# tangxyw/RecAlgorithm

Measured on AMD Instinct MI355X. Metric: CTR examples/sec (train step fwd+bwd+TF1-Adam), batch 4096/GPU, 26 fields x emb16, higher is better.
Workload: dtype f32; 1 GPU; DCN 3-layer CrossNet + MLP 512,256,128; 26 fields x emb16; batch 4096/GPU; data_batches=32, global_batch=4096, fields=26, emb_dim=16, embedding_rows=2790871, launch=hipGraph replay, parallelism=single

## Files before the change

### recalgorithm_amd/_lib.py

```python
from __future__ import annotations

import ctypes
import os
import re

from . import _abi
from ._abi import RecalgoError

_HERE = os.path.dirname(os.path.abspath(__file__))
LIB_PATH = os.environ.get("RECALGO_HIP_LIB") or os.path.join(_HERE, "librecalgo_hip.so")

P = ctypes.c_void_p


def _versioned(header: str):
    abi = _abi.read(header)
    defines = [c for c in abi.constants if re.fullmatch(r"RECALGO_(?:[A-Z0-9]+_)?ABI_VERSION", c)]
    queries = [f for f in abi.functions if re.fullmatch(r"recalgo_(?:[a-z0-9]+_)?abi_version", f)]
    if len(defines) != 1 or queries != [defines[0].lower()]:
        raise RecalgoError(f"include/{header}: a header of HEADERS has exactly one RECALGO_[<KEY>_]ABI_VERSION define and the "
                           f"one function recalgo_[<key>_]abi_version of the same key; found {defines} and {queries}")
    abi.version, abi.version_query = abi.constants[defines[0]], queries[0]
    abi.label = defines[0][len("RECALGO_"):-len("_VERSION")].replace("_", " ")
    return abi


HEADERS = {h: _versioned(h) for h in ("recalgo.h", "recalgo_cgc.h", "recalgo_wide.h", "recalgo_bst.h",
                                              "recalgo_res.h")}
MORE_HEADERS = {"recalgo_dien.h": _versioned("recalgo_dien.h")}
SERVING_HEADERS = {h: _versioned(h) for h in ("recalgo_serve.h", "recalgo_metrics.h", "recalgo_sumstep.h",
                                                      "recalgo_ragged.h", "recalgo_afm.h", "recalgo_feed.h")}
ABI = HEADERS["recalgo.h"]
SIGNATURES = ABI.functions
STRUCTS = ABI.structs
CONSTANTS = ABI.constants
ABI_VERSION = ABI.version
_lib = None


def all_headers() -> dict:
    return {**HEADERS, **MORE_HEADERS}


def every_header() -> dict:
    return {**all_headers(), **SERVING_HEADERS}

# ... 38 lines not shown
```

### recalgorithm_amd/algorithm/DCN/dcn.py

```python
from __future__ import annotations

import os
from typing import Tuple

import torch

from ... import feature_column as fc
from ... import flags, nn, ops
from ...estimator import (Estimator, EvalSpec, ModeKeys, RunConfig, TrainSpec, train_and_evaluate)
from ...model_tail import finish_model_fn
from ...variables import variable_scope
from .. import _common as common
from ..utils import eval_input_fn, parse_example, train_input_fn
from .cross_layer import cross_network

flags.DEFINE_string("model_dir", "./model_dir", "Directory where model parameters, graph, etc are saved")
flags.DEFINE_string("output_dir", "./output_dir", "Directory where pb file are saved")
flags.DEFINE_string("train_data", "../../dataset/wechat_algo_data1/tfrecord/train.tfrecord", "Path to the train data")
flags.DEFINE_string("eval_data", "../../dataset/wechat_algo_data1/tfrecord/test.tfrecord", "Path to the evaluation data")
flags.DEFINE_string("vocabulary_dir", "../../dataset/wechat_algo_data1/vocabulary/", "Folder where the vocabulary file is stored")
flags.DEFINE_integer("num_epochs", 1, "Epoch of training phase")
flags.DEFINE_integer("train_steps", 10000, "Number of (global) training steps to perform")
flags.DEFINE_integer("shuffle_buffer_size", 10000, "Dataset shuffle buffer size")
flags.DEFINE_integer("num_parallel_readers", -1, "Number of parallel readers for training data")
# ... 51 lines not shown

def dcn_model_fn(features, labels, mode, params):
    with variable_scope("dense_input"):
        dense_cols = params.get("dense_feature_columns") or []
        dense_input = fc.input_layer(features, dense_cols) if dense_cols else None
    with variable_scope("category_input"):
        if dense_input is None and int(params["num_cross_layer"]) > 0:
            with ops.gather_feeds_cross() as lz:
                category_input = fc.input_layer(features, params["category_feature_columns"])
                lz.keep(category_input)
        else:
            category_input = fc.input_layer(features, params["category_feature_columns"])
    concat_all = category_input if dense_input is None else torch.cat([dense_input, category_input], dim=-1)

    join = nn.GradJoin() if int(params["num_cross_layer"]) > 0 and len(params["hidden_units"]) > 0 else None
    with variable_scope("cross_part"):
        cross_vec = cross_network(concat_all, params["num_cross_layer"], grad_join=join)
    ops.flush_lazy_gathers()

    with variable_scope("dnn_part"):
        dnn_vec = concat_all
        for i, unit in enumerate(params["hidden_units"]):
            dnn_vec = nn.dense(dnn_vec, unit, activation="relu", name=f"dnn_dense_{i}", grad_join=join if i == 0 else None,
                               last_hidden=(i == len(params["hidden_units"]) - 1))

    with variable_scope("output_part"):
        output = nn.concat([cross_vec, dnn_vec], axis=-1)
        logit = nn.dense(output, 1, activation=None)

    return finish_model_fn(mode, logit, labels, params,
                           predictions=lambda prob: {"logit": logit, "probabilities": prob})


def main(unused_argv):
    global total_feature_columns, label_feature_columns
    dense_cols, category_cols, label_feature_columns = create_feature_columns()
    total_feature_columns = dense_cols + category_cols
    params = {
        "category_feature_columns": category_cols,
# ... 46 lines not shown
```

### recalgorithm_amd/csrc/cross.hip

```cpp
#include "common.h"
#include "cross_bwd.h"

namespace {

constexpr int kFwdThreads = 256;
constexpr int kBwdThreads = 512;
constexpr int kBwdWaves = kBwdThreads / 64;
constexpr int kMaxPartialRows = 256;

using recalgo_cross::wave_sum_n;

struct GatherSrc {
    const int64_t* ids;
    const float4* arena;
    const int64_t* row_base;
    unsigned F, K4;
};

template <int NV, int L>
__global__ __launch_bounds__(kFwdThreads) void cross_stack_fwd_kernel(
    float* __restrict__ x0, unsigned x_stride, const float4* __restrict__ w,
    const float4* __restrict__ b, unsigned B, unsigned d4, float* __restrict__ out,
    unsigned out_stride, GatherSrc gs) {
    const unsigned lane = threadIdx.x & 63;
    const unsigned wave = (blockIdx.x * kFwdThreads + threadIdx.x) >> 6;
    const unsigned nwaves = (gridDim.x * kFwdThreads) >> 6;

    float4 wv[L][NV], Bv[NV];
    float red[2 * L];
#pragma unroll
    for (int v = 0; v < NV; ++v) Bv[v] = f4_zero();
#pragma unroll
    for (int l = 0; l < L; ++l) {
        float acc = 0.f;
#pragma unroll
        for (int v = 0; v < NV; ++v) {
            unsigned idx = lane + v * 64;
            wv[l][v] = idx < d4 ? w[l * d4 + idx] : f4_zero();
            acc += f4_dot(Bv[v], wv[l][v]);
            if (idx < d4) Bv[v] = f4_add(Bv[v], b[l * d4 + idx]);
        }
        red[L + l] = acc;
    }

    for (unsigned ex = wave; ex < B; ex += nwaves) {
        float4* xr = reinterpret_cast<float4*>(x0 + (size_t)ex * x_stride);
        float4 xv[NV];
        if (gs.ids != nullptr) {
            long long id[NV];
#pragma unroll
            for (int v = 0; v < NV; ++v) {
                const unsigned idx = lane + v * 64;
                id[v] = idx < d4 ? gs.ids[(size_t)ex * gs.F + idx / gs.K4] : -1;
            }
#pragma unroll
            for (int v = 0; v < NV; ++v) {
                const unsigned idx = lane + v * 64, f = idx / gs.K4, q = idx - f * gs.K4;
                xv[v] = id[v] >= 0 ? gs.arena[(size_t)(gs.row_base[f] + id[v]) * gs.K4 + q] : f4_zero();
                if (idx < d4) xr[idx] = xv[v];
            }
        } else {
#pragma unroll
            for (int v = 0; v < NV; ++v) {
                unsigned idx = lane + v * 64;
                xv[v] = idx < d4 ? xr[idx] : f4_zero();
            }
        }
        float r[2 * L];
#pragma unroll
        for (int l = 0; l < L; ++l) {
            float acc = 0.f;
#pragma unroll
            for (int v = 0; v < NV; ++v) acc += f4_dot(xv[v], wv[l][v]);
            r[l] = acc;
            r[L + l] = red[L + l];
        }
        wave_sum_n<2 * L>(r);
        float c = 1.f;
#pragma unroll
        for (int l = 0; l < L; ++l) c += fmaf(c, r[l], r[L + l]);
        float4* orow = reinterpret_cast<float4*>(out + (size_t)ex * out_stride);
#pragma unroll
        for (int v = 0; v < NV; ++v) {
            unsigned idx = lane + v * 64;
            if (idx < d4) orow[idx] = f4_fma(xv[v], c, Bv[v]);
        }
    }
}

template <int NV, int L>
__global__ __launch_bounds__(kBwdThreads) void cross_stack_bwd_kernel(
    const float* __restrict__ x0, unsigned x_stride, const float4* __restrict__ w,
    const float4* __restrict__ b, const float* __restrict__ g, unsigned g_stride,
    const float* __restrict__ g_x0_extra, unsigned B, unsigned d4, float* __restrict__ dx0,
    float* __restrict__ partials) {
    extern __shared__ __attribute__((aligned(16))) float smem[];
    recalgo_cross::cross_stack_bwd_block<NV, L, kBwdWaves>(x0, x_stride, w, b, g, g_stride, g_x0_extra, B, d4, dx0, partials, blockIdx.x,
                                                          gridDim.x, smem);
}

template <int NV>
__global__ __launch_bounds__(kFwdThreads) void cross_layer_fwd_kernel(
// ... 269 lines not shown
```

### recalgorithm_amd/csrc/dense.hip

```cpp
#include <cstdlib>

#include "common.h"
#include "cross_bwd.h"
#include "act.h"
#include "tile_v2.h"
#include "dropout.h"
#include "slab_sum.h"

namespace {

using f32x16 = __attribute__((ext_vector_type(16))) float;

constexpr int kThreads = 256;
constexpr int BM = 64, BN = 64, BK = 32;
constexpr int kLdRC = BK + 1;
constexpr int kLdRM = 64;
constexpr int kBufFloats = 64 * tv2::kLdRC;

struct Operand {
    const float* p;
    const float* mask;
    int ld;
    int vec;
    int bytes;
// ... 222 lines not shown
    Segment seg[2];
    int nseg;
    const float* bias;
    int relu;
    float* y;
    int ldy;
    int M, N;
    float* bn_partials;
    const float* act_alpha;
    int act_kind;
    float* z;
    int vec_store;
    recalgo_drop::Spec drop;
};

template <bool FAST>
__global__ __launch_bounds__(kThreads) void dense_fwd_kernel(FwdArgs P) {
    __shared__ __attribute__((aligned(16))) float As[kStages * kBufFloats];
    __shared__ __attribute__((aligned(16))) float Bs[kStages * kBufFloats];
    const int tn_count = (P.N + BN - 1) / BN;
    const int tile = xcd_swizzle(blockIdx.x, gridDim.x);
    const int m0 = (tile / tn_count) * BM, n0 = (tile % tn_count) * BN;
    f32x16 acc, acc1;
#pragma unroll
    for (int r = 0; r < 16; ++r) acc[r] = acc1[r] = 0.f;
    float4 unused = f4_zero();
    const int lane = threadIdx.x & 63, wave = threadIdx.x >> 6;
    const int hi = lane >> 5, l32 = lane & 31;
    const bool rowwise = FAST && P.vec_store && P.bn_partials == nullptr;
    const int c4 = n0 + (wave & 1) * 32 + (lane & 7) * 4;
    float4 bias4 = f4_zero();
    if (rowwise && P.bias && c4 < P.N) bias4 = *reinterpret_cast<const float4*>(P.bias + c4);
    for (int s = 0; s < P.nseg; ++s)
        tile_mainloop<true, false, FAST, false, false, false>(P.seg[s], m0, n0, P.M, P.N, 0, P.seg[s].n_red, As, Bs, acc, acc1, unused);
    acc += acc1;
    const int col = n0 + (wave & 1) * 32 + l32;
    const bool dropping = recalgo_drop::enabled(P.drop);
    const recalgo_drop::Key dkey = dropping ? recalgo_drop::make_key(P.drop) : recalgo_drop::Key{0u, 0u};
    if (rowwise) {
        const int r0 = m0 + (wave >> 1) * 32;
        tv2::tile_rows(As + wave * tv2::kTileScratch, acc, [&](int, int row, int, float4 v) {
            v = f4_add(v, bias4);
            if (P.relu) v = make_float4(fmaxf(v.x, 0.f), fmaxf(v.y, 0.f), fmaxf(v.z, 0.f), fmaxf(v.w, 0.f));
            if (r0 + row < P.M && c4 < P.N) {
                if (dropping) {
                    const float4 f = recalgo_drop::factor4(P.drop, dkey, (uint32_t)(r0 + row) * (uint32_t)P.N + (uint32_t)c4);
                    v = make_float4(v.x * f.x, v.y * f.y, v.z * f.z, v.w * f.w);
                }
                *reinterpret_cast<float4*>(P.y + (size_t)(r0 + row) * P.ldy + c4) = v;
            }
        });
        return;
    }
    if (P.bn_partials == nullptr) {
        if (col >= P.N) return;
        const float bv = P.bias ? P.bias[col] : 0.f;
#pragma unroll
        for (int r = 0; r < 16; ++r) {
            const int row = m0 + (wave >> 1) * 32 + (r & 3) + 8 * (r >> 2) + 4 * hi;
            if (row < P.M) {
                float v = acc[r] + bv;
                if (P.relu) v = fmaxf(v, 0.f);
                if (dropping) v *= recalgo_drop::factor(P.drop, dkey, (uint32_t)row * (uint32_t)P.N + (uint32_t)col);
                P.y[(size_t)row * P.ldy + col] = v;
            }
        }
// ... 41 lines not shown
#pragma unroll
    for (int r = 0; r < 16; ++r) {
        const int row = m0 + (wave >> 1) * 32 + (r & 3) + 8 * (r >> 2) + 4 * hi;
        const float dlt = vals[r] - mean;
        if (cok && row < P.M) q = fmaf(dlt, dlt, q);
    }
    q += __shfl_xor(q, 32, 64);
    __syncthreads();
    if (hi == 0) red[(wave >> 1) * 64 + cl] = q;
    __syncthreads();
    if ((wave >> 1) == 0 && hi == 0 && cok) {
        float* prow = P.bn_partials + (size_t)(m0 / BM) * 2 * P.N;
        prow[col] = mean;
        prow[P.N + col] = red[cl] + red[64 + cl];
    }
}

struct DgradArgs {
    Segment seg;
    const float* c_in;
    float beta;
    int ldc;
    float* dx;
    int lddx;
    int M, K;
    int accumulate;
    int tiles_per_block;
    int vec_store;
    const float* dx_mask;
    int ld_mask;
// ... 343 lines not shown
    P.seg[0] = Segment{operand(x, nullptr, ldx, M, K), operand(w, nullptr, N, K, N), K};
    P.seg[1] = Segment{operand(x2, nullptr, ldx2, M, K2), operand(w2, nullptr, N, K2, N), K2};
    P.nseg = x2 ? 2 : 1;
    P.bias = bias; P.relu = relu; P.y = y; P.ldy = ldy; P.M = M; P.N = N;
    P.bn_partials = bn_partials;
    P.act_alpha = act_alpha; P.act_kind = act_kind == RECALGO_ACT_NONE ? 0 : 1 + act_kind; P.z = z;
    P.vec_store = (aligned16(y) && ldy % 4 == 0 && N % 4 == 0 && (bias == nullptr || aligned16(bias))) ? 1 : 0;
    P.drop = recalgo_drop::from_abi(drop);
    const int grid = cdiv(M, BM) * cdiv(N, BN);
    const bool fast = fast_rc(P.seg[0].a, K) && fast_rm(P.seg[0].b, N) && fast_rc(P.seg[1].a, K2) && fast_rm(P.seg[1].b, N);
    if (fast) hipLaunchKernelGGL(dense_fwd_kernel<true>, dim3(grid), dim3(kThreads), 0, as_stream(stream), P);
    else hipLaunchKernelGGL(dense_fwd_kernel<false>, dim3(grid), dim3(kThreads), 0, as_stream(stream), P);
    RECALGO_RETURN_LAST();
}

static bool build_dgrad(DgradArgs& P, const float* g, int ldg, const float* y_mask, const float* w, int M, int N, int K,
                        const float* c_in, int ldc, float beta, float* dx, int lddx, int accumulate) {
    if (!(M >= 0 && N > 0 && K > 0 && dx != nullptr && lddx >= K)) return false;
    if (!(g != nullptr && ldg >= N && w != nullptr)) return false;
    if (!(c_in == nullptr || ldc >= K)) return false;
    P.seg = Segment{operand(g, y_mask, ldg, M, N), operand(w, nullptr, N, K, N), N};
    P.c_in = c_in; P.beta = beta; P.ldc = ldc; P.dx = dx; P.lddx = lddx; P.M = M; P.K = K; P.accumulate = accumulate;
    P.tiles_per_block = 1;
    P.bn_x = P.bn_mean = P.bn_rstd = nullptr; P.bn_partials = nullptr;
    P.vec_store = (aligned16(dx) && lddx % 4 == 0 && K % 4 == 0 && (c_in == nullptr || (aligned16(c_in) && ldc % 4 == 0))) ? 1 : 0;
    P.dx_mask = nullptr; P.ld_mask = 0;
    return true;
}
static bool dgrad_fast(const DgradArgs& P) { return fast_rc(P.seg.a, P.seg.n_red) && fast_rc(P.seg.b, P.seg.n_red); }

// ... 300 lines not shown
```

### recalgorithm_amd/csrc/tile_v2.h

```cpp
#pragma once
#include "common.h"

namespace tv2 {

using f32x16 = __attribute__((ext_vector_type(16))) float;

constexpr int kThreads = 256;
constexpr int BK = 32;
constexpr int kLdRC = 36;
constexpr int kStages = 3;
constexpr int kOOB = (int)0x80000000u;

struct Operand {
    const float* p;
    const float* mask;
    int ld;
    int bytes;
};

template <bool RC, int W>
struct Geom {
    static constexpr int T = 64 * W;
    static constexpr int kFloats = RC ? T * kLdRC : BK * T;
    static constexpr int kLoads = 2 * W;
// ... 44 lines not shown
            const int o = red[j] + c * BK < red_end ? off[j] + c * step_b : kOOB;
            st.v[j] = __builtin_bit_cast(float4, __builtin_amdgcn_raw_buffer_load_b128(rs, o, 0, 0));
            if constexpr (MASK) st.m[j] = __builtin_bit_cast(float4, __builtin_amdgcn_raw_buffer_load_b128(rm, o, 0, 0));
        }
    }
    static __device__ __forceinline__ float4 value(const StageRegs<MASK, G::kLoads>& st, int j) {
        if constexpr (MASK) return relu_mask4(st.v[j], st.m[j]);
        else return st.v[j];
    }
    static __device__ __forceinline__ void store(float* __restrict__ S, const StageRegs<MASK, G::kLoads>& st, int j) {
        const int u = threadIdx.x + kThreads * j;
        float* d;
        if constexpr (RC) d = S + (u >> 3) * kLdRC + (u & 7) * 4;
        else d = S + (u / G::U) * G::T + (u % G::U) * 4;
        *reinterpret_cast<float4*>(d) = value(st, j);
    }
};

template <int W>
struct Frag {
    float x[4][W];
};

template <bool RC, int W>
__device__ __forceinline__ void read_item(const float* __restrict__ S, int wb, int l32, int hi, int g, int item, Frag<W>& f) {
    if constexpr (RC) {
        const float4 q = *reinterpret_cast<const float4*>(S + (wb + 32 * item + l32) * kLdRC + 8 * g + 4 * hi);
        f.x[0][item] = q.x; f.x[1][item] = q.y; f.x[2][item] = q.z; f.x[3][item] = q.w;
    } else {
        const float* p = S + (8 * g + 4 * hi + item) * Geom<false, W>::T + wb + W * l32;
        if constexpr (W == 1) f.x[item][0] = p[0];
        else if constexpr (W == 2) { const float2 q = *reinterpret_cast<const float2*>(p); f.x[item][0] = q.x; f.x[item][1] = q.y; }
        else { const float4 q = *reinterpret_cast<const float4*>(p); f.x[item][0] = q.x; f.x[item][1] = q.y; f.x[item][2] = q.z; f.x[item][3] = q.w; }
    }
}
template <bool RC, int W> constexpr int frag_items() { return RC ? W : 4; }

template <bool RC, int W>
__device__ __forceinline__ int idx_of(int sub, int lane_idx) { return RC ? 32 * sub + lane_idx : W * lane_idx + sub; }

template <bool A_RC, bool B_RC, int WM, int WN, bool MASK_A, bool MASK_B, bool COLSUM, bool EXACT, bool TWO = false>
__device__ __forceinline__ void mainloop(const Operand& A, const Operand& B, int m0, int n0, int M, int N, int red_begin,
                                         int red_end, float* __restrict__ As, float* __restrict__ Bs,
                                         f32x16 (&acc)[WM][WN], float4& colsum, f32x16 (*accb)[WN] = nullptr) {
    using GA = Geom<A_RC, WM>;
    using GB = Geom<B_RC, WN>;
    using SA = Stager<A_RC, WM, MASK_A, EXACT>;
    using SB = Stager<B_RC, WN, MASK_B, EXACT>;
    constexpr int nLA = GA::kLoads, nLB = GB::kLoads, nL = nLA + nLB;
    constexpr int nFA = frag_items<A_RC, WM>(), nFB = frag_items<B_RC, WN>(), nF = nFA + nFB;
    constexpr int G = 4 * WM * WN;
    static_assert(nL <= G, "one load / store item per slot");
    const int lane = threadIdx.x & 63, wave = threadIdx.x >> 6;
    const int hi = lane >> 5, l32 = lane & 31;
    const int wbA = (wave >> 1) * 32 * WM, wbB = (wave & 1) * 32 * WN;
    const int nchunks = (red_end - red_begin + BK - 1) / BK;
    if (nchunks <= 0) return;
    SA ga;
    SB gb;
    ga.init(A, m0, red_begin, M, red_end);
    gb.init(B, n0, red_begin, N, red_end);
    StageRegs<MASK_A, nLA> sa[2];
// ... 123 lines not shown
```

### recalgorithm_amd/ops.py

```python
from __future__ import annotations

import ctypes
from typing import Callable, NamedTuple, Optional, Tuple

import torch
from torch.autograd import Function

from . import _lib, sparse
from .variables import EmbeddingArena, Variable, VariableStore

_C = _lib.CONSTANTS
_ACT = {"prelu": _C["RECALGO_ACT_PRELU"], "dice": _C["RECALGO_ACT_DICE"]}
_ACT_NONE = _C["RECALGO_ACT_NONE"]
_Live, _ColSum, _DenseSplit = (_lib.STRUCTS[n] for n in ("recalgo_live_t", "recalgo_colsum_t", "recalgo_dense_split_t"))
_CDrop, _AdamArena = _lib.STRUCTS["recalgo_dropout_t"], _lib.STRUCTS["recalgo_adam_arena_t"]


def _lib_():
    return _lib.load()


def _p(t: Optional[torch.Tensor]):
    return None if t is None else ctypes.c_void_p(t.data_ptr())

# ... 20 lines not shown


_ws_cache = {}


_lazy_gathers: list = []
_cross_rider = None
_wgrad_rider = None
_dense_pending = []
_colsum_pending = []
_dlogit_partials = {}
_parked_l2 = []


def discard_step_work() -> None:
    global _wgrad_rider, _cross_rider
    _lazy_gathers.clear()
    _wgrad_rider = _cross_rider = None
    _dense_pending.clear()
    _colsum_pending.clear()
    _dlogit_partials.clear()
    _parked_l2.clear()
    _bst_shared.clear()


def anchor_store(anchor):
    return getattr(anchor, "_recalgo_store", None)


def _flush(arena) -> None:
    f = getattr(arena, "flush_grad", None)
    if f is not None:
# ... 55 lines not shown
        self._kept = False
        return self

    def keep(self, x) -> None:
        self._kept = (len(_lazy_gathers) == 1 and isinstance(x, torch.Tensor) and _lazy_gathers[0][0] is x)

    def __exit__(self, *exc):
        global _lazy_gather_on
        _lazy_gather_on = self._prev
        if not self._kept:
            flush_lazy_gathers()
        return False


def flush_lazy_gathers() -> None:
    while _lazy_gathers:
        out, ids, arena, row_base = _lazy_gathers.pop()
        out._recalgo_lazy_gather = None
        B, F = ids.shape
        _lib_().recalgo_embedding_gather_fwd(_p(ids), _p(arena.weight), _p(row_base), B, F, arena.K, _p(out), F * arena.K, 0,
                                             _stream(ids))


def _take_lazy_gather(x0: torch.Tensor):
    lz = getattr(x0, "_recalgo_lazy_gather", None)
    if lz is not None:
        for i, ent in enumerate(_lazy_gathers):
            if ent[0] is x0:
                _lazy_gathers.pop(i)
                break
        x0._recalgo_lazy_gather = None
    flush_lazy_gathers()
    return lz


class _GatherFn(Function):
# ... 253 lines not shown
    _chk(ids, torch.int64, "ids")
    if getattr(arena, "sharding", None) is not None:
        from . import parallel
        plan, staged, ident = _staged(arena, parallel.global_rows(ids, row_base), store)
        staged_w1 = parallel.StagedArena(plan, w1_arena, store, torch.is_grad_enabled())
        return _DeepFMSparseFn.apply(store.anchor, ident.reshape(ids.shape), staged, staged_w1, bias,
                                     torch.zeros_like(row_base), False)
    return _DeepFMSparseFn.apply(store.anchor, ids, arena, w1_arena, bias, row_base, torch.is_grad_enabled())


def _pad4(t: torch.Tensor) -> torch.Tensor:
    pad = (-t.shape[-1]) % 4
    return t if pad == 0 else torch.nn.functional.pad(t, (0, pad))


class _CrossFn(Function):
    @staticmethod
    def forward(ctx, anchor, x0, w: Variable, b: Variable, grad_join):
        ctx.grad_join = grad_join
        B, d = x0.shape
        L = w.data.shape[0]
        lz = _take_lazy_gather(x0)
        x0p, wp, bp = _pad4(x0), _pad4(w.data.reshape(L, d)), _pad4(b.data.reshape(L, d))
        dp = x0p.shape[1]
        out = torch.empty(B, dp, device=x0.device, dtype=torch.float32)
        if lz is not None and dp == d and x0.is_contiguous():
            ids, arena, row_base = lz
            _lib_().recalgo_gather_cross_fwd(_p(ids), _p(arena.weight), _p(row_base), B, ids.shape[1], arena.K, _p(wp), _p(bp), L,
                                             _p(x0), d, _p(out), dp, _stream(x0))
        else:
            if lz is not None:
                ids, arena, row_base = lz
                _lib_().recalgo_embedding_gather_fwd(_p(ids), _p(arena.weight), _p(row_base), B, ids.shape[1], arena.K, _p(x0),
                                                     ids.shape[1] * arena.K, 0, _stream(ids))
                x0p = _pad4(x0)
            _lib_().recalgo_cross_fwd(_p(x0p), dp, _p(wp), _p(bp), B, dp, L, _p(out), dp, _stream(x0))
        ctx.vars = (w, b)
        ctx.d = d
        ctx.save_for_backward(x0p)
        return out if dp == d else out[:, :d]

# ... 48 lines not shown
        if dp != d:
            w.grad.copy_(dw[:, :d].reshape(w.grad.shape))
            b.grad.copy_(db[:, :d].reshape(b.grad.shape))
            dx0 = dx0[:, :d]
        if extra is not None and not fused_extra:
            dx0 = dx0 + extra.reshape(dx0.shape)
        if stale_dx is not None:
            dx0 = dx0 - stale_dx.reshape(dx0.shape)
        return None, dx0, None, None, None


def cross_stack(store, x0: torch.Tensor, w: Variable, b: Variable, grad_join=None) -> torch.Tensor:
    if store.building:
        return torch.zeros_like(x0)
    _chk(x0, torch.float32, "x0")
    out = _CrossFn.apply(store.anchor, x0, w, b, grad_join)
    if grad_join is not None and out.grad_fn is not None:
        out._recalgo_cross_node = out.grad_fn
    return out


class _CrossLayerFn(Function):

    @staticmethod
    def forward(ctx, anchor, x0, xl, w: Variable, b: Variable):
        B, d = x0.shape
        x0p, xlp = _pad4(x0), _pad4(xl)
        wp, bp = _pad4(w.data.reshape(1, d)), _pad4(b.data.reshape(1, d))
        dp = x0p.shape[1]
        out = torch.empty(B, dp, device=x0.device, dtype=torch.float32)
# ... 581 lines not shown
              bn_partials: Optional[torch.Tensor] = None, drop: Optional["DropSpec"] = None) -> torch.Tensor:
    x, w = _mat(x, "x"), _mat(w, "w")
    M, K = x.shape
    N = w.shape[1]
    if w.shape[0] != K or w.stride(0) != N:
        raise ValueError("dense_fwd: w must be a contiguous [K, N] matrix")
    if x2 is not None:
        x2, w2 = _mat(x2, "x2"), _mat(w2, "w2")
        if w2.shape != (x2.shape[1], N) or w2.stride(0) != N or x2.shape[0] != M:
            raise ValueError("dense_fwd: second operand pair does not match")
    y = torch.empty(M, N, device=x.device, dtype=torch.float32)
    if bn_partials is not None and (tuple(bn_partials.shape) != (bn_partial_rows(M), 2 * N) or not bn_partials.is_contiguous()):
        raise ValueError("dense_fwd: bn_partials must be a contiguous [bn_partial_rows(M), 2 N] tensor")
    if drop is not None:
        drop.check_mask((M, N))
    cd, _keep = _cdrop(drop)
    _lib_().recalgo_dense_fwd(
        _p(x), x.stride(0), _p(w), K, _p(x2), 0 if x2 is None else x2.stride(0), _p(w2), 0 if x2 is None else x2.shape[1],
        _p(bias), M, N, int(relu), _ACT_NONE, None, None, _p(y), N, _p(bn_partials), cd, _stream(x))
    return y


def dense_fwd_act(x: torch.Tensor, w: torch.Tensor, bias: Optional[torch.Tensor], kind: int, alpha: torch.Tensor,
                  bn_partials: torch.Tensor):
    x, w = _mat(x, "x"), _mat(w, "w")
    M, K = x.shape
    N = w.shape[1]
    if w.shape[0] != K or w.stride(0) != N:
        raise ValueError("dense_fwd_act: w must be a contiguous [K, N] matrix")
    if tuple(bn_partials.shape) != (bn_partial_rows(M), 2 * N) or not bn_partials.is_contiguous():
# ... 1520 lines not shown
```

Measured before the change: 21.05 million examples/s.

## Fuse embedding gather and cross stack into first dense layer forward kernel

```diff
diff --git a/include/recalgo_gatherdense.h b/include/recalgo_gatherdense.h
--- /dev/null
+++ b/include/recalgo_gatherdense.h
@@ -0,0 +1,25 @@
+#ifndef RECALGO_GATHERDENSE_H_
+#define RECALGO_GATHERDENSE_H_
+
+#include <stdint.h>
+
+#ifdef __cplusplus
+extern "C" {
+#endif
+
+typedef void* recalgo_stream_t;
+
+#define RECALGO_GATHERDENSE_ABI_VERSION 1
+int recalgo_gatherdense_abi_version(void);
+
+int recalgo_dense_fwd_gather_cross_supported(int64_t arena_rows, int F, int K, int N, int L);
+int recalgo_dense_fwd_gather_cross(const int64_t* ids, const float* arena, int64_t arena_rows, const int64_t* row_base, int B, int F,
+                                   int K, const float* w, const float* bias, int N, int relu, float* y, int y_pitch,
+                                   const float* cross_w, const float* cross_b, int L, float* x0, int x0_pitch, float* out,
+                                   int out_pitch, recalgo_stream_t stream);
+
+#ifdef __cplusplus
+}
+#endif
+
+#endif
diff --git a/recalgorithm_amd/_lib.py b/recalgorithm_amd/_lib.py
--- a/recalgorithm_amd/_lib.py
+++ b/recalgorithm_amd/_lib.py
@@ -29,7 +29,8 @@
                                               "recalgo_res.h")}
 MORE_HEADERS = {"recalgo_dien.h": _versioned("recalgo_dien.h")}
 SERVING_HEADERS = {h: _versioned(h) for h in ("recalgo_serve.h", "recalgo_metrics.h", "recalgo_sumstep.h",
-                                                      "recalgo_ragged.h", "recalgo_afm.h", "recalgo_feed.h")}
+                                                      "recalgo_ragged.h", "recalgo_afm.h", "recalgo_feed.h",
+                                                      "recalgo_gatherdense.h")}
 ABI = HEADERS["recalgo.h"]
 SIGNATURES = ABI.functions
 STRUCTS = ABI.structs
diff --git a/recalgorithm_amd/algorithm/DCN/dcn.py b/recalgorithm_amd/algorithm/DCN/dcn.py
--- a/recalgorithm_amd/algorithm/DCN/dcn.py
+++ b/recalgorithm_amd/algorithm/DCN/dcn.py
@@ -89,15 +89,20 @@
     concat_all = category_input if dense_input is None else torch.cat([dense_input, category_input], dim=-1)
 
     join = nn.GradJoin() if int(params["num_cross_layer"]) > 0 and len(params["hidden_units"]) > 0 else None
-    with variable_scope("cross_part"):
-        cross_vec = cross_network(concat_all, params["num_cross_layer"], grad_join=join)
+    hidden = list(params["hidden_units"])
+    with ops.cross_rides_dense():
+        with variable_scope("cross_part"):
+            cross_vec = cross_network(concat_all, params["num_cross_layer"], grad_join=join)
+        with variable_scope("dnn_part"):
+            dnn_vec = concat_all
+            if hidden:
+                dnn_vec = nn.dense(dnn_vec, hidden[0], activation="relu", name="dnn_dense_0", grad_join=join,
+                                   last_hidden=(len(hidden) == 1))
     ops.flush_lazy_gathers()
 
     with variable_scope("dnn_part"):
-        dnn_vec = concat_all
-        for i, unit in enumerate(params["hidden_units"]):
-            dnn_vec = nn.dense(dnn_vec, unit, activation="relu", name=f"dnn_dense_{i}", grad_join=join if i == 0 else None,
-                               last_hidden=(i == len(params["hidden_units"]) - 1))
+        for i, unit in enumerate(hidden[1:], start=1):
+            dnn_vec = nn.dense(dnn_vec, unit, activation="relu", name=f"dnn_dense_{i}", last_hidden=(i == len(hidden) - 1))
 
     with variable_scope("output_part"):
         output = nn.concat([cross_vec, dnn_vec], axis=-1)
diff --git a/recalgorithm_amd/csrc/cross.hip b/recalgorithm_amd/csrc/cross.hip
--- a/recalgorithm_amd/csrc/cross.hip
+++ b/recalgorithm_amd/csrc/cross.hip
@@ -1,5 +1,6 @@
 #include "common.h"
 #include "cross_bwd.h"
+#include "cross_fwd.h"
 
 namespace {
 
@@ -10,82 +11,14 @@
 
 using recalgo_cross::wave_sum_n;
 
-struct GatherSrc {
-    const int64_t* ids;
-    const float4* arena;
-    const int64_t* row_base;
-    unsigned F, K4;
-};
+using recalgo_cross::GatherSrc;
 
 template <int NV, int L>
 __global__ __launch_bounds__(kFwdThreads) void cross_stack_fwd_kernel(
     float* __restrict__ x0, unsigned x_stride, const float4* __restrict__ w,
     const float4* __restrict__ b, unsigned B, unsigned d4, float* __restrict__ out,
     unsigned out_stride, GatherSrc gs) {
-    const unsigned lane = threadIdx.x & 63;
-    const unsigned wave = (blockIdx.x * kFwdThreads + threadIdx.x) >> 6;
-    const unsigned nwaves = (gridDim.x * kFwdThreads) >> 6;
-
-    float4 wv[L][NV], Bv[NV];
-    float red[2 * L];
-#pragma unroll
-    for (int v = 0; v < NV; ++v) Bv[v] = f4_zero();
-#pragma unroll
-    for (int l = 0; l < L; ++l) {
-        float acc = 0.f;
-#pragma unroll
-        for (int v = 0; v < NV; ++v) {
-            unsigned idx = lane + v * 64;
-            wv[l][v] = idx < d4 ? w[l * d4 + idx] : f4_zero();
-            acc += f4_dot(Bv[v], wv[l][v]);
-            if (idx < d4) Bv[v] = f4_add(Bv[v], b[l * d4 + idx]);
-        }
-        red[L + l] = acc;
-    }
-
-    for (unsigned ex = wave; ex < B; ex += nwaves) {
-        float4* xr = reinterpret_cast<float4*>(x0 + (size_t)ex * x_stride);
-        float4 xv[NV];
-        if (gs.ids != nullptr) {
-            long long id[NV];
-#pragma unroll
-            for (int v = 0; v < NV; ++v) {
-                const unsigned idx = lane + v * 64;
-                id[v] = idx < d4 ? gs.ids[(size_t)ex * gs.F + idx / gs.K4] : -1;
-            }
-#pragma unroll
-            for (int v = 0; v < NV; ++v) {
-                const unsigned idx = lane + v * 64, f = idx / gs.K4, q = idx - f * gs.K4;
-                xv[v] = id[v] >= 0 ? gs.arena[(size_t)(gs.row_base[f] + id[v]) * gs.K4 + q] : f4_zero();
-                if (idx < d4) xr[idx] = xv[v];
-            }
-        } else {
-#pragma unroll
-            for (int v = 0; v < NV; ++v) {
-                unsigned idx = lane + v * 64;
-                xv[v] = idx < d4 ? xr[idx] : f4_zero();
-            }
-        }
-        float r[2 * L];
-#pragma unroll
-        for (int l = 0; l < L; ++l) {
-            float acc = 0.f;
-#pragma unroll
-            for (int v = 0; v < NV; ++v) acc += f4_dot(xv[v], wv[l][v]);
-            r[l] = acc;
-            r[L + l] = red[L + l];
-        }
-        wave_sum_n<2 * L>(r);
-        float c = 1.f;
-#pragma unroll
-        for (int l = 0; l < L; ++l) c += fmaf(c, r[l], r[L + l]);
-        float4* orow = reinterpret_cast<float4*>(out + (size_t)ex * out_stride);
-#pragma unroll
-        for (int v = 0; v < NV; ++v) {
-            unsigned idx = lane + v * 64;
-            if (idx < d4) orow[idx] = f4_fma(xv[v], c, Bv[v]);
-        }
-    }
+    recalgo_cross::cross_stack_fwd_block<NV, L, kFwdThreads / 64>(x0, x_stride, w, b, B, d4, out, out_stride, gs, blockIdx.x, gridDim.x);
 }
 
 template <int NV, int L>
diff --git a/recalgorithm_amd/csrc/cross_fwd.h b/recalgorithm_amd/csrc/cross_fwd.h
--- /dev/null
+++ b/recalgorithm_amd/csrc/cross_fwd.h
@@ -0,0 +1,85 @@
+#pragma once
+#include "common.h"
+#include "cross_bwd.h"
+
+namespace recalgo_cross {
+
+struct GatherSrc {
+    const int64_t* ids;
+    const float4* arena;
+    const int64_t* row_base;
+    unsigned F, K4;
+};
+
+template <int NV, int L, int WAVES>
+__device__ __forceinline__ void cross_stack_fwd_block(
+    float* __restrict__ x0, unsigned x_stride, const float4* __restrict__ w,
+    const float4* __restrict__ b, unsigned B, unsigned d4, float* __restrict__ out,
+    unsigned out_stride, const GatherSrc& gs, unsigned block, unsigned nblocks) {
+    const unsigned lane = threadIdx.x & 63;
+    const unsigned wave = block * WAVES + (threadIdx.x >> 6);
+    const unsigned nwaves = nblocks * WAVES;
+
+    float4 wv[L][NV], Bv[NV];
+    float red[2 * L];
+#pragma unroll
+    for (int v = 0; v < NV; ++v) Bv[v] = f4_zero();
+#pragma unroll
+    for (int l = 0; l < L; ++l) {
+        float acc = 0.f;
+#pragma unroll
+        for (int v = 0; v < NV; ++v) {
+            unsigned idx = lane + v * 64;
+            wv[l][v] = idx < d4 ? w[l * d4 + idx] : f4_zero();
+            acc += f4_dot(Bv[v], wv[l][v]);
+            if (idx < d4) Bv[v] = f4_add(Bv[v], b[l * d4 + idx]);
+        }
+        red[L + l] = acc;
+    }
+
+    for (unsigned ex = wave; ex < B; ex += nwaves) {
+        float4* xr = reinterpret_cast<float4*>(x0 + (size_t)ex * x_stride);
+        float4 xv[NV];
+        if (gs.ids != nullptr) {
+            long long id[NV];
+#pragma unroll
+            for (int v = 0; v < NV; ++v) {
+                const unsigned idx = lane + v * 64;
+                id[v] = idx < d4 ? gs.ids[(size_t)ex * gs.F + idx / gs.K4] : -1;
+            }
+#pragma unroll
+            for (int v = 0; v < NV; ++v) {
+                const unsigned idx = lane + v * 64, f = idx / gs.K4, q = idx - f * gs.K4;
+                xv[v] = id[v] >= 0 ? gs.arena[(size_t)(gs.row_base[f] + id[v]) * gs.K4 + q] : f4_zero();
+                if (idx < d4) xr[idx] = xv[v];
+            }
+        } else {
+#pragma unroll
+            for (int v = 0; v < NV; ++v) {
+                unsigned idx = lane + v * 64;
+                xv[v] = idx < d4 ? xr[idx] : f4_zero();
+            }
+        }
+        float r[2 * L];
+#pragma unroll
+        for (int l = 0; l < L; ++l) {
+            float acc = 0.f;
+#pragma unroll
+            for (int v = 0; v < NV; ++v) acc += f4_dot(xv[v], wv[l][v]);
+            r[l] = acc;
+            r[L + l] = red[L + l];
+        }
+        wave_sum_n<2 * L>(r);
+        float c = 1.f;
+#pragma unroll
+        for (int l = 0; l < L; ++l) c += fmaf(c, r[l], r[L + l]);
+        float4* orow = reinterpret_cast<float4*>(out + (size_t)ex * out_stride);
+#pragma unroll
+        for (int v = 0; v < NV; ++v) {
+            unsigned idx = lane + v * 64;
+            if (idx < d4) orow[idx] = f4_fma(xv[v], c, Bv[v]);
+        }
+    }
+}
+
+}
diff --git a/recalgorithm_amd/csrc/dense.hip b/recalgorithm_amd/csrc/dense.hip
--- a/recalgorithm_amd/csrc/dense.hip
+++ b/recalgorithm_amd/csrc/dense.hip
@@ -2,10 +2,12 @@
 
 #include "common.h"
 #include "cross_bwd.h"
+#include "cross_fwd.h"
 #include "act.h"
 #include "tile_v2.h"
 #include "dropout.h"
 #include "slab_sum.h"
+#include "../../include/recalgo_gatherdense.h"
 
 namespace {
 
@@ -260,6 +262,22 @@
     recalgo_drop::Spec drop;
 };
 
+__device__ __forceinline__ void store_rows_bias_relu(float* __restrict__ T, const f32x16& acc, float4 bias4, int relu, int r0, int c4,
+                                                     int M, int N, float* __restrict__ y, int ldy, bool dropping,
+                                                     const recalgo_drop::Spec& drop, const recalgo_drop::Key& dkey) {
+    tv2::tile_rows(T, acc, [&](int, int row, int, float4 v) {
+        v = f4_add(v, bias4);
+        if (relu) v = make_float4(fmaxf(v.x, 0.f), fmaxf(v.y, 0.f), fmaxf(v.z, 0.f), fmaxf(v.w, 0.f));
+        if (r0 + row < M && c4 < N) {
+            if (dropping) {
+                const float4 f = recalgo_drop::factor4(drop, dkey, (uint32_t)(r0 + row) * (uint32_t)N + (uint32_t)c4);
+                v = make_float4(v.x * f.x, v.y * f.y, v.z * f.z, v.w * f.w);
+            }
+            *reinterpret_cast<float4*>(y + (size_t)(r0 + row) * ldy + c4) = v;
+        }
+    });
+}
+
 template <bool FAST>
 __global__ __launch_bounds__(kThreads) void dense_fwd_kernel(FwdArgs P) {
     __shared__ __attribute__((aligned(16))) float As[kStages * kBufFloats];
@@ -284,18 +302,8 @@
     const bool dropping = recalgo_drop::enabled(P.drop);
     const recalgo_drop::Key dkey = dropping ? recalgo_drop::make_key(P.drop) : recalgo_drop::Key{0u, 0u};
     if (rowwise) {
-        const int r0 = m0 + (wave >> 1) * 32;
-        tv2::tile_rows(As + wave * tv2::kTileScratch, acc, [&](int, int row, int, float4 v) {
-            v = f4_add(v, bias4);
-            if (P.relu) v = make_float4(fmaxf(v.x, 0.f), fmaxf(v.y, 0.f), fmaxf(v.z, 0.f), fmaxf(v.w, 0.f));
-            if (r0 + row < P.M && c4 < P.N) {
-                if (dropping) {
-                    const float4 f = recalgo_drop::factor4(P.drop, dkey, (uint32_t)(r0 + row) * (uint32_t)P.N + (uint32_t)c4);
-                    v = make_float4(v.x * f.x, v.y * f.y, v.z * f.z, v.w * f.w);
-                }
-                *reinterpret_cast<float4*>(P.y + (size_t)(r0 + row) * P.ldy + c4) = v;
-            }
-        });
+        store_rows_bias_relu(As + wave * tv2::kTileScratch, acc, bias4, P.relu, m0 + (wave >> 1) * 32, c4, P.M, P.N, P.y, P.ldy,
+                             dropping, P.drop, dkey);
         return;
     }
     if (P.bn_partials == nullptr) {
@@ -367,6 +375,64 @@
         prow[col] = mean;
         prow[P.N + col] = red[cl] + red[64 + cl];
     }
+}
+
+struct GatherFwdArgs {
+    tv2::GatherOperand a;
+    tv2::Operand w;
+    const float* bias;
+    int relu;
+    float* y;
+    int ldy, M, N;
+    recalgo_cross::GatherSrc gs;
+    float* x0;
+    float* out;
+    const float4* cw;
+    const float4* cb;
+    unsigned x_stride, out_stride, rider_blocks;
+};
+
+template <int NV, int L, bool EXACT>
+__global__ __launch_bounds__(kThreads) void gather_rider_dense_fwd_kernel(GatherFwdArgs P) {
+    __shared__ __attribute__((aligned(16))) float As[kStages * kBufFloats];
+    __shared__ __attribute__((aligned(16))) float Bs[kStages * kBufFloats];
+    __shared__ int rowoff[tv2::kGatherTable];
+    int b = (int)blockIdx.x;
+    if (b < (int)P.rider_blocks) {
+        recalgo_cross::cross_stack_fwd_block<NV, L, kThreads / 64>(P.x0, P.x_stride, P.cw, P.cb, (unsigned)P.M, (unsigned)(P.a.d / 4), P.out,
+                                                                  P.out_stride, P.gs, (unsigned)b, P.rider_blocks);
+        return;
+    }
+    b -= (int)P.rider_blocks;
+    const int tiles = (int)gridDim.x - (int)P.rider_blocks;
+    const bool carry = P.rider_blocks == 0, carry_first = ((b >> 8) & 1) == 0;
+    if (carry && carry_first)
+        recalgo_cross::cross_stack_fwd_block<NV, L, kThreads / 64>(P.x0, P.x_stride, P.cw, P.cb, (unsigned)P.M, (unsigned)(P.a.d / 4), P.out,
+                                                                  P.out_stride, P.gs, (unsigned)b, (unsigned)tiles);
+    const int tn_count = (P.N + BN - 1) / BN;
+    const int tile = xcd_swizzle(b, tiles);
+    const int m0 = (tile / tn_count) * BM, n0 = (tile % tn_count) * BN;
+    f32x16 acc, acc1;
+#pragma unroll
+    for (int r = 0; r < 16; ++r) acc[r] = acc1[r] = 0.f;
+    float4 unused = f4_zero();
+    const int lane = threadIdx.x & 63, wave = threadIdx.x >> 6;
+    const int c4 = n0 + (wave & 1) * 32 + (lane & 7) * 4;
+    float4 bias4 = f4_zero();
+    if (P.bias && c4 < P.N) bias4 = *reinterpret_cast<const float4*>(P.bias + c4);
+    tv2::GatherOperand a = P.a;
+    a.table = rowoff;
+    tv2::f32x16 (&acc2)[1][1] = *reinterpret_cast<tv2::f32x16 (*)[1][1]>(&acc);
+    tv2::f32x16 (*accb)[1] = reinterpret_cast<tv2::f32x16 (*)[1]>(&acc1);
+    tv2::mainloop<true, false, 1, 1, false, false, false, EXACT, true, tv2::GatherStager, tv2::GatherOperand>(a, P.w, m0, n0, P.M, P.N, 0, a.d, As,
+                                                                                                           Bs, acc2, unused, accb);
+    acc += acc1;
+    const recalgo_drop::Spec nodrop{nullptr, nullptr, 0u, 0u, 0u, 0.f};
+    store_rows_bias_relu(As + wave * tv2::kTileScratch, acc, bias4, P.relu, m0 + (wave >> 1) * 32, c4, P.M, P.N, P.y, P.ldy, false, nodrop,
+                         recalgo_drop::Key{0u, 0u});
+    if (carry && !carry_first)
+        recalgo_cross::cross_stack_fwd_block<NV, L, kThreads / 64>(P.x0, P.x_stride, P.cw, P.cb, (unsigned)P.M, (unsigned)(P.a.d / 4), P.out,
+                                                                  P.out_stride, P.gs, (unsigned)b, (unsigned)tiles);
 }
 
 struct DgradArgs {
@@ -740,6 +806,70 @@
     RECALGO_RETURN_LAST();
 }
 
+RECALGO_EXPORT int recalgo_gatherdense_abi_version(void) { return RECALGO_GATHERDENSE_ABI_VERSION; }
+
+RECALGO_EXPORT int recalgo_dense_fwd_gather_cross_supported(int64_t arena_rows, int F, int K, int N, int L) {
+    if (!(K >= 4 && K % 4 == 0 && F >= 1 && F <= tv2::kGatherMaxF && (int64_t)F * K <= 512 && L >= 1 && L <= 4)) return 0;
+    if (!(arena_rows >= 0 && arena_rows * K * (int64_t)sizeof(float) < (1ll << 31))) return 0;
+    if (!(N > 0 && N % 4 == 0 && (int64_t)F * K * N * (int64_t)sizeof(float) < (1ll << 31) - (1ll << 24))) return 0;
+    return 1;
+}
+
+#ifndef RECALGO_FWD_RIDER
+#define RECALGO_FWD_RIDER 0
+#endif
+static int fwd_rider_blocks(int B, int tiles) {
+    const int per_wave = cdiv(B, kThreads / 64), loop = cdiv(B, 16) > 256 ? 256 : cdiv(B, 16);
+    if (RECALGO_FWD_RIDER == 1) return loop;
+    if (RECALGO_FWD_RIDER == 2) return per_wave;
+    if (tiles + per_wave <= kResidentBlocks) return per_wave;
+    if (tiles + loop <= kResidentBlocks) return loop;
+    return 0;
+}
+
+RECALGO_EXPORT int recalgo_dense_fwd_gather_cross(const int64_t* ids, const float* arena, int64_t arena_rows, const int64_t* row_base,
+                                                  int B, int F, int K, const float* w, const float* bias, int N, int relu, float* y,
+                                                  int ldy, const float* cross_w, const float* cross_b, int L, float* x0, int x_stride,
+                                                  float* out, int out_stride, recalgo_stream_t stream) {
+    RECALGO_REQUIRE(B >= 0 && recalgo_dense_fwd_gather_cross_supported(arena_rows, F, K, N, L));
+    const int d = F * K;
+    RECALGO_REQUIRE(ldy >= N && ldy % 4 == 0);
+    RECALGO_REQUIRE(x_stride >= d && x_stride % 4 == 0);
+    RECALGO_REQUIRE(out_stride >= d && out_stride % 4 == 0);
+    RECALGO_REQUIRE(ids != nullptr && arena != nullptr && row_base != nullptr && w != nullptr && y != nullptr);
+    RECALGO_REQUIRE(cross_w != nullptr && cross_b != nullptr && x0 != nullptr && out != nullptr);
+    RECALGO_REQUIRE(aligned16(ids, arena, row_base, w, bias, y) && aligned16(cross_w, cross_b, x0, out));
+    if (B == 0) return 0;
+    GatherFwdArgs P;
+    P.a = tv2::GatherOperand{arena, (int)(arena_rows * K * (int64_t)sizeof(float)), ids, row_base, F, K, d, nullptr};
+    P.w = tv2::Operand{w, nullptr, N, (int)((int64_t)d * N * (int64_t)sizeof(float))};
+    P.bias = bias; P.relu = relu; P.y = y; P.ldy = ldy; P.M = B; P.N = N;
+    P.gs = recalgo_cross::GatherSrc{ids, reinterpret_cast<const float4*>(arena), row_base, (unsigned)F, (unsigned)(K / 4)};
+    P.x0 = x0; P.out = out;
+    P.cw = reinterpret_cast<const float4*>(cross_w); P.cb = reinterpret_cast<const float4*>(cross_b);
+    P.x_stride = (unsigned)x_stride; P.out_stride = (unsigned)out_stride;
+    P.rider_blocks = (unsigned)fwd_rider_blocks(B, cdiv(B, BM) * cdiv(N, BN));
+    const dim3 grid(P.rider_blocks + cdiv(B, BM) * cdiv(N, BN)), block(kThreads);
+    hipStream_t st = as_stream(stream);
+    const bool exact = d % BK == 0;
+#define GD_LAUNCH(NV, LL)                                                                                                 \
+    do {                                                                                                                  \
+        if (exact) hipLaunchKernelGGL((gather_rider_dense_fwd_kernel<NV, LL, true>), grid, block, 0, st, P);               \
+        else hipLaunchKernelGGL((gather_rider_dense_fwd_kernel<NV, LL, false>), grid, block, 0, st, P);                    \
+    } while (0)
+#define GD_L(NV)                                \
+    switch (L) {                                \
+        case 1: GD_LAUNCH(NV, 1); break;        \
+        case 2: GD_LAUNCH(NV, 2); break;        \
+        case 3: GD_LAUNCH(NV, 3); break;        \
+        default: GD_LAUNCH(NV, 4); break;       \
+    }
+    if (d / 4 <= 64) { GD_L(1) } else { GD_L(2) }
+#undef GD_L
+#undef GD_LAUNCH
+    RECALGO_RETURN_LAST();
+}
+
 static bool build_dgrad(DgradArgs& P, const float* g, int ldg, const float* y_mask, const float* w, int M, int N, int K,
                         const float* c_in, int ldc, float beta, float* dx, int lddx, int accumulate) {
     if (!(M >= 0 && N > 0 && K > 0 && dx != nullptr && lddx >= K)) return false;
diff --git a/recalgorithm_amd/csrc/tile_v2.h b/recalgorithm_amd/csrc/tile_v2.h
--- a/recalgorithm_amd/csrc/tile_v2.h
+++ b/recalgorithm_amd/csrc/tile_v2.h
@@ -82,6 +82,76 @@
         if constexpr (RC) d = S + (u >> 3) * kLdRC + (u & 7) * 4;
         else d = S + (u / G::U) * G::T + (u % G::U) * 4;
         *reinterpret_cast<float4*>(d) = value(st, j);
+    }
+};
+
+struct GatherOperand {
+    const float* arena;
+    int bytes;
+    const int64_t* ids;
+    const int64_t* row_base;
+    int F, K, d;
+    int* table;
+};
+
+constexpr int kGatherMaxF = 32;
+constexpr int kGatherTable = 64 * kGatherMaxF;
+
+struct GatherStager {
+    using G = Geom<true, 1>;
+    __amdgpu_buffer_rsrc_t rs;
+    const int* tab;
+    int rowF[G::kLoads];
+    int nxt[G::kLoads];
+    int r0, K, kinv, F, d;
+
+    __device__ __forceinline__ int field_of(int r) const { return (int)(((unsigned)r * (unsigned)kinv) >> 20); }
+    __device__ __forceinline__ int entry(int j, int r) const {
+        const int f = field_of(r);
+        return tab[rowF[j] + (f < F ? f : F - 1)];
+    }
+    __device__ __forceinline__ void init(const GatherOperand& op, int m0, int, int M, int) {
+        const int t = threadIdx.x;
+        int* __restrict__ table = op.table;
+        rs = __builtin_amdgcn_make_buffer_rsrc(const_cast<float*>(op.arena), (short)0, op.bytes, 0x00020000);
+        tab = table;
+        K = op.K; F = op.F; d = op.d;
+        kinv = ((1 << 20) + op.K - 1) / op.K;
+        const int n = 64 * op.F, valid = (M - m0 < 64 ? M - m0 : 64) * op.F;
+        const int64_t* src = op.ids + (size_t)m0 * op.F;
+        const int row_bytes = op.K * (int)sizeof(float);
+        constexpr int kPer = kGatherTable / kThreads;
+        const unsigned finv = ((1u << 16) + op.F - 1) / op.F;
+        int64_t idv[kPer], rbv[kPer];
+#pragma unroll
+        for (int i = 0; i < kPer; ++i) {
+            const int e = t + kThreads * i;
+            const int f = e - (int)(((unsigned)e * finv) >> 16) * op.F;
+            idv[i] = e < valid ? src[e] : -1;
+            rbv[i] = e < n ? op.row_base[f] : 0;
+        }
+#pragma unroll
+        for (int i = 0; i < kPer; ++i) {
+            const int e = t + kThreads * i;
+            if (e < n) table[e] = idv[i] >= 0 ? (int)((rbv[i] + idv[i]) * (int64_t)row_bytes) : kOOB;
+        }
+        r0 = (t & 7) * 4;
+#pragma unroll
+        for (int j = 0; j < G::kLoads; ++j) rowF[j] = ((t + kThreads * j) >> 3) * op.F;
+        __syncthreads();
+#pragma unroll
+        for (int j = 0; j < G::kLoads; ++j) nxt[j] = entry(j, r0);
+    }
+    __device__ __forceinline__ void issue(int c, int j, StageRegs<false, G::kLoads>& st) {
+        const int r = r0 + c * BK;
+        const int q = r - field_of(r) * K;
+        const int o = r < d ? nxt[j] + q * (int)sizeof(float) : kOOB;
+        st.v[j] = __builtin_bit_cast(float4, __builtin_amdgcn_raw_buffer_load_b128(rs, o, 0, 0));
+        nxt[j] = entry(j, r + BK);
+    }
+    static __device__ __forceinline__ float4 value(const StageRegs<false, G::kLoads>& st, int j) { return st.v[j]; }
+    static __device__ __forceinline__ void store(float* __restrict__ S, const StageRegs<false, G::kLoads>& st, int j) {
+        Stager<true, 1, false, false>::store(S, st, j);
     }
 };
 
@@ -107,13 +177,13 @@
 template <bool RC, int W>
 __device__ __forceinline__ int idx_of(int sub, int lane_idx) { return RC ? 32 * sub + lane_idx : W * lane_idx + sub; }
 
-template <bool A_RC, bool B_RC, int WM, int WN, bool MASK_A, bool MASK_B, bool COLSUM, bool EXACT, bool TWO = false>
-__device__ __forceinline__ void mainloop(const Operand& A, const Operand& B, int m0, int n0, int M, int N, int red_begin,
+template <bool A_RC, bool B_RC, int WM, int WN, bool MASK_A, bool MASK_B, bool COLSUM, bool EXACT, bool TWO = false,
+          class SA = Stager<A_RC, WM, MASK_A, EXACT>, class AOp = Operand>
+__device__ __forceinline__ void mainloop(const AOp& A, const Operand& B, int m0, int n0, int M, int N, int red_begin,
                                          int red_end, float* __restrict__ As, float* __restrict__ Bs,
                                          f32x16 (&acc)[WM][WN], float4& colsum, f32x16 (*accb)[WN] = nullptr) {
     using GA = Geom<A_RC, WM>;
     using GB = Geom<B_RC, WN>;
-    using SA = Stager<A_RC, WM, MASK_A, EXACT>;
     using SB = Stager<B_RC, WN, MASK_B, EXACT>;
     constexpr int nLA = GA::kLoads, nLB = GB::kLoads, nL = nLA + nLB;
     constexpr int nFA = frag_items<A_RC, WM>(), nFB = frag_items<B_RC, WN>(), nF = nFA + nFB;
diff --git a/recalgorithm_amd/ops.py b/recalgorithm_amd/ops.py
--- a/recalgorithm_amd/ops.py
+++ b/recalgorithm_amd/ops.py
@@ -58,8 +58,9 @@
 
 
 def discard_step_work() -> None:
-    global _wgrad_rider, _cross_rider
+    global _wgrad_rider, _cross_rider, _parked_cross, _cross_ride_on
     _lazy_gathers.clear()
+    _parked_cross, _cross_ride_on = None, False
     _wgrad_rider = _cross_rider = None
     _dense_pending.clear()
     _colsum_pending.clear()
@@ -145,12 +146,68 @@
 
 
 def flush_lazy_gathers() -> None:
+    flush_parked_cross()
     while _lazy_gathers:
         out, ids, arena, row_base = _lazy_gathers.pop()
         out._recalgo_lazy_gather = None
         B, F = ids.shape
         _lib_().recalgo_embedding_gather_fwd(_p(ids), _p(arena.weight), _p(row_base), B, F, arena.K, _p(out), F * arena.K, 0,
                                              _stream(ids))
+
+
+CROSS_RIDES_DENSE = True
+_cross_ride_on = False
+_cross_ride_grad = False
+_parked_cross = None
+cross_ride_counters = {"rides": 0, "flushes": 0}
+
+
+class cross_rides_dense:
+
+    def __enter__(self):
+        global _cross_ride_on
+        self._prev, _cross_ride_on = _cross_ride_on, bool(CROSS_RIDES_DENSE)
+        return self
+
+    def __exit__(self, *exc):
+        global _cross_ride_on
+        _cross_ride_on = self._prev
+        flush_parked_cross()
+        return False
+
+
+def _ptrs_aligned16(*ts) -> bool:
+    return all(t is None or t.data_ptr() % 16 == 0 for t in ts)
+
+
+def _gather_dense_supported(arena, F: int, N: int, L: int) -> bool:
+    return bool(_lib_().recalgo_dense_fwd_gather_cross_supported(int(arena.weight.shape[0]), int(F), int(arena.K), int(N), int(L)))
+
+
+def flush_parked_cross() -> None:
+    global _parked_cross
+    rec, _parked_cross = _parked_cross, None
+    if rec is None:
+        return
+    cross_ride_counters["flushes"] += 1
+    x0, ids, arena, row_base, w, b, L, out = rec
+    B, d = x0.shape
+    _lib_().recalgo_gather_cross_fwd(_p(ids), _p(arena.weight), _p(row_base), B, ids.shape[1], arena.K, _p(w), _p(b), L, _p(x0), d,
+                                     _p(out), d, _stream(x0))
+
+
+def _take_parked_cross(x: torch.Tensor, w: torch.Tensor, bias, y: torch.Tensor, plain_relu: bool):
+    global _parked_cross
+    rec = _parked_cross
+    if rec is None:
+        return None
+    x0, ids, arena = rec[0], rec[1], rec[2]
+    same = x.data_ptr() == x0.data_ptr() and tuple(x.shape) == tuple(x0.shape) and x.stride() == x0.stride()
+    if (plain_relu and same and _gather_dense_supported(arena, ids.shape[1], w.shape[1], rec[6]) and _ptrs_aligned16(w, bias, y)):
+        _parked_cross = None
+        return rec
+    flush_parked_cross()
+    return None
 
 
 def _take_lazy_gather(x0: torch.Tensor):
@@ -434,6 +491,16 @@
     return t if pad == 0 else torch.nn.functional.pad(t, (0, pad))
 
 
+def _park_cross(x0, lz, w, b, L, out) -> bool:
+    global _parked_cross
+    ids, arena, row_base = lz
+    if not (_cross_ride_grad and _gather_dense_supported(arena, ids.shape[1], 4, L)
+            and _ptrs_aligned16(ids, arena.weight, row_base, w, b, x0, out)):
+        return False
+    _parked_cross = (x0, ids, arena, row_base, w, b, L, out)
+    return True
+
+
 class _CrossFn(Function):
     @staticmethod
     def forward(ctx, anchor, x0, w: Variable, b: Variable, grad_join):
@@ -444,7 +511,12 @@
         x0p, wp, bp = _pad4(x0), _pad4(w.data.reshape(L, d)), _pad4(b.data.reshape(L, d))
         dp = x0p.shape[1]
         out = torch.empty(B, dp, device=x0.device, dtype=torch.float32)
-        if lz is not None and dp == d and x0.is_contiguous():
+        parked = _cross_ride_on and lz is not None and dp == d and x0.is_contiguous() and _park_cross(x0, lz, wp, bp, L, out)
+        if _cross_ride_on and not parked:
+            cross_ride_counters["flushes"] += 1
+        if parked:
+            pass
+        elif lz is not None and dp == d and x0.is_contiguous():
             ids, arena, row_base = lz
             _lib_().recalgo_gather_cross_fwd(_p(ids), _p(arena.weight), _p(row_base), B, ids.shape[1], arena.K, _p(wp), _p(bp), L,
                                              _p(x0), d, _p(out), dp, _stream(x0))
@@ -523,6 +595,8 @@
     if store.building:
         return torch.zeros_like(x0)
     _chk(x0, torch.float32, "x0")
+    global _cross_ride_grad
+    _cross_ride_grad = torch.is_grad_enabled()
     out = _CrossFn.apply(store.anchor, x0, w, b, grad_join)
     if grad_join is not None and out.grad_fn is not None:
         out._recalgo_cross_node = out.grad_fn
@@ -1134,6 +1208,14 @@
         raise ValueError("dense_fwd: bn_partials must be a contiguous [bn_partial_rows(M), 2 N] tensor")
     if drop is not None:
         drop.check_mask((M, N))
+    rec = _take_parked_cross(x, w, bias, y, bool(relu) and x2 is None and bn_partials is None and drop is None)
+    if rec is not None:
+        x0, ids, arena, row_base, cw, cb, L, out = rec
+        cross_ride_counters["rides"] += 1
+        _lib_().recalgo_dense_fwd_gather_cross(
+            _p(ids), _p(arena.weight), int(arena.weight.shape[0]), _p(row_base), M, ids.shape[1], arena.K, _p(w), _p(bias), N, 1,
+            _p(y), N, _p(cw), _p(cb), L, _p(x0), K, _p(out), K, _stream(x))
+        return y
     cd, _keep = _cdrop(drop)
     _lib_().recalgo_dense_fwd(
         _p(x), x.stride(0), _p(w), K, _p(x2), 0 if x2 is None else x2.stride(0), _p(w2), 0 if x2 is None else x2.shape[1],
```

New measurement: 21.19 million examples/s, median of 6. Within noise of the previous version (+0.6%).
